# FrancisTheCat/raytracing_c

Measured on NVIDIA B200. Metric: Msamples/s (pixel*spp/s), helmet.glb 1920x1080, higher is better.
Workload: dtype f32

## Files before the change

### raytracing_c_b200/csrc/rt_stages.cuh

```cuda
#pragma once

#include <cuda_runtime.h>
#include <math_constants.h>

#include "rt_device.cuh"
#include "rt_fastdiv.h"
#include "rt_trace.cuh"
#include "rt_shade.cuh"

#if defined(RT_FAST) && RT_FAST
#define RT_KN(name) name##_fast
#else
#define RT_KN(name) name
#endif

#ifndef RT_TRACE_MIN_BLOCKS
#define RT_TRACE_MIN_BLOCKS 3
#endif
#ifndef RT_TRACE_MIN_BLOCKS_PRIMARY
#define RT_TRACE_MIN_BLOCKS_PRIMARY 4
#endif
#ifndef RT_TRACE_MIN_BLOCKS_WIDE
#define RT_TRACE_MIN_BLOCKS_WIDE 4
#endif
#ifndef RT_TRACE_WIDE_BOUNCES
#define RT_TRACE_WIDE_BOUNCES 2
#endif
#define RT_FULL 0xffffffffu
#ifndef RT_EMIT_ONE_ATOMIC
#define RT_EMIT_ONE_ATOMIC 1
#endif
#ifndef RT_BATCH_MAX
#define RT_BATCH_MAX 256u
#endif
#ifndef RT_ROOT_STEP_AT_REFILL
#define RT_ROOT_STEP_AT_REFILL 1
#endif

enum { Q_RAYS = 0, Q_FETCH = 1, Q_HITS = 2, Q_MISSES = 3, Q_STRIDE = 4 };

struct PathQueues {
  float4 *ray_a, *ray_b;
  float4 *hit_a, *hit_b, *hit_h;
  float4 *miss_a;
  float4 *tint, *emis;
  float4 *rad;
  unsigned *counts;
};

struct StageParams {
  SceneDev   scene;
  PathQueues q;
  int        width, height, tiles_x, tiles_y;
  int        split_rank, split_world, chunks_x;
  unsigned   n_tiles;
  int        sample0, n_samples;
  int        bounce, max_bounces;
  uint32_t   user_seed;
  unsigned   n_paths;
  RT_FastDiv div_samples, div_tiles_x, div_chunks_x;
  int        accumulate;
  float     *accum;
  float     *per_sample;
  int        per_sample_stride, per_sample_offset;
  int       *hit_ids;
  unsigned long long *counters;
  unsigned long long *counters_ex;
};

__device__ __forceinline__ float fract1(float v) { return v - floorf(v); }
__device__ __forceinline__ float hash12(float px, float py) {
  float a = fract1(px * 0.1031f);
  float b = fract1(py * 0.1031f);
  float c = fract1(px * 0.1031f);
  float k = 33.33f;
  float d = a * (b + k) + b * (c + k) + c * (a + k);
  return fract1((a + b + d * 2.0f) * (c + d));
}

__device__ __forceinline__ void tile_origin(const StageParams &P, unsigned tile, int &x0, int &y0) {
  if (P.split_world <= 1) {
    const unsigned row = rt_fastdiv(tile, P.div_tiles_x, (unsigned)P.tiles_x);
    x0 = (int)(tile - row * (unsigned)P.tiles_x) * 8;
    y0 = (int)row * 4;
  } else {
    const unsigned chunk = (tile >> 5) * (unsigned)P.split_world + (unsigned)P.split_rank, t = tile & 31u;
    const unsigned row = rt_fastdiv(chunk, P.div_chunks_x, (unsigned)P.chunks_x);
    x0 = (int)(chunk - row * (unsigned)P.chunks_x) * 32 + (int)(t & 3u) * 8;
    y0 = (int)row * 32 + (int)(t >> 2) * 4;
  }
}

#ifndef RT_PATH_LAYOUT
#define RT_PATH_LAYOUT 1
#endif
__device__ __forceinline__ void path_pixel(const StageParams &P, unsigned path, int &px, int &py, int &ls) {
#if RT_PATH_LAYOUT == 1
  const unsigned pix = rt_fastdiv(path, P.div_samples, (unsigned)P.n_samples);
  ls = (int)(path - pix * (unsigned)P.n_samples);
  const unsigned in_tile = pix & 31u, tile = pix >> 5;
#else
  unsigned in_tile = path & 31u, rest = path >> 5;
  unsigned tile = rest / (unsigned)P.n_samples;
  ls = (int)(rest - tile * (unsigned)P.n_samples);
#endif
  int x0, y0;
  tile_origin(P, tile, x0, y0);
  px = x0 + (int)(in_tile & 7u);
  py = y0 + (int)(in_tile >> 3);
}

__device__ __forceinline__ void add_counter(unsigned long long *counters, int k, unsigned v) {
  v += __shfl_xor_sync(RT_FULL, v, 16);
  v += __shfl_xor_sync(RT_FULL, v, 8);
  v += __shfl_xor_sync(RT_FULL, v, 4);
  v += __shfl_xor_sync(RT_FULL, v, 2);
  v += __shfl_xor_sync(RT_FULL, v, 1);
  if ((threadIdx.x & 31) == 0 && v) atomicAdd(&counters[k], (unsigned long long)v);
}

__device__ __forceinline__ unsigned warp_append(unsigned *count, bool want, unsigned lane) {
  const unsigned mask = __ballot_sync(RT_FULL, want);
  unsigned base = 0;
  if (lane == 0 && mask) base = atomicAdd(count, (unsigned)__popc(mask));
  base = __shfl_sync(RT_FULL, base, 0);
  return base + (unsigned)__popc(mask & ((1u << lane) - 1u));
}

#ifndef RT_MIN_BATCH
#define RT_MIN_BATCH 4u
#endif
#ifndef RT_REFILL_MIN_PRIMARY
#define RT_REFILL_MIN_PRIMARY 32
#endif
#ifndef RT_REFILL_MIN_BOUNCE
#define RT_REFILL_MIN_BOUNCE 20
#endif

template <bool PRIMARY, int MIN_BLOCKS = (PRIMARY ? RT_TRACE_MIN_BLOCKS_PRIMARY : RT_TRACE_MIN_BLOCKS)>
__global__ void __launch_bounds__(RT_BLOCK, MIN_BLOCKS)
RT_KN(rt_trace_kernel)(const __grid_constant__ StageParams P) {
  extern __shared__ float4 level_store[];
  const SceneDev &sc = P.scene;
  const unsigned lane = threadIdx.x & 31u;
  const unsigned lt_mask = (1u << lane) - 1u;
  float4 *levels = level_store + threadIdx.x;
  unsigned *counts = P.q.counts + P.bounce * Q_STRIDE;
  const unsigned n_in = PRIMARY ? P.n_paths : counts[Q_RAYS];
  unsigned c_rays = 0, c_nodes = 0, c_leaves = 0, c_accepts = 0, c_root_miss = 0;

  const float inv_w = 1.0f / (float)P.width, inv_h = 1.0f / (float)P.height;
  const float aspect = (float)P.width / (float)P.height;

  RayWalk w;
  w.flags = 0; w.leaf = -1; w.hit_slot = -1;
  bool     exhausted = false;
  unsigned q = 0, range_next = 0, range_end = 0;
  uint32_t seed0 = 0;
  const unsigned total_warps = gridDim.x * (RT_BLOCK / 32);
  unsigned batch = (n_in / (total_warps * 4u)) & ~31u;
  if (batch > RT_BATCH_MAX) batch = RT_BATCH_MAX;
  if (batch < 32u) {
    batch = (n_in + total_warps - 1u) / total_warps;
    if (batch < RT_MIN_BATCH) batch = RT_MIN_BATCH;
    if (batch > 32u) batch = 32u;
  }

  unsigned walking = 0;
  for (;;) {
    if (walking == 0 || (!exhausted && __popc(~walking) >= (PRIMARY ? RT_REFILL_MIN_PRIMARY : RT_REFILL_MIN_BOUNCE))) {
      const bool fin = (w.flags & (WALK_RAY | WALK_LIVE)) == WALK_RAY;
      const bool is_hit = fin && w.hit_slot >= 0;
      const bool is_miss = fin && w.hit_slot < 0;
      if (__any_sync(RT_FULL, fin)) {
        unsigned path = q;
        uint32_t rng = seed0;
        if (fin) {
          if (PRIMARY) {
            if (P.hit_ids) {
              int px, py, ls;
              path_pixel(P, q, px, py, ls);
              if (ls == 0) P.hit_ids[py * P.width + px] = w.hit_slot;
            }
          } else {
            const float4 b = P.q.ray_b[q];
            path = __float_as_uint(b.z);
            rng  = __float_as_uint(b.w);
          }
        }
#if RT_EMIT_ONE_ATOMIC
        const unsigned hmask = __ballot_sync(RT_FULL, is_hit), mmask = __ballot_sync(RT_FULL, is_miss);
        unsigned long long both = 0;
        if (lane == 0)
          both = atomicAdd(reinterpret_cast<unsigned long long *>(&counts[Q_HITS]),
                           (unsigned long long)__popc(hmask) | ((unsigned long long)__popc(mmask) << 32));
        both = __shfl_sync(RT_FULL, both, 0);
        const unsigned hpos = (unsigned)both + (unsigned)__popc(hmask & lt_mask);
        const unsigned mpos = (unsigned)(both >> 32) + (unsigned)__popc(mmask & lt_mask);
#else
        const unsigned hpos = warp_append(&counts[Q_HITS], is_hit, lane);
        const unsigned mpos = warp_append(&counts[Q_MISSES], is_miss, lane);
#endif
        if (is_hit) {
          P.q.hit_a[hpos] = make_float4(w.ox, w.oy, w.oz, w.dx);
          P.q.hit_b[hpos] = make_float4(w.dy, w.dz, __uint_as_float(path), __uint_as_float(rng));
          P.q.hit_h[hpos] = make_float4(w.hit_t, w.hit_u, w.hit_v, __int_as_float(w.hit_slot));
        }
        if (is_miss) {
          P.q.miss_a[mpos] = make_float4(w.dx, w.dy, w.dz, __uint_as_float(path));
        }
        if (fin) w.flags = 0;
      }
      if (!exhausted) {
        const unsigned idle = ~walking;
        if (range_next >= range_end) {
          unsigned base = 0;
          if (lane == 0) base = atomicAdd(&counts[Q_FETCH], batch);
          base = __shfl_sync(RT_FULL, base, 0);
          exhausted = base >= n_in;
          range_next = base;
          range_end = exhausted ? base : min(base + batch, n_in);
          if (batch > 32u) {
            const unsigned share = ((n_in - range_end) / (total_warps * 2u)) & ~31u;
            batch = share < 32u ? 32u : (share < batch ? share : batch);
          }
        }
        const unsigned take = min((unsigned)__popc(idle), range_end - range_next);
        const unsigned rank = (unsigned)__popc(idle & lt_mask);
        if ((idle >> lane & 1u) && rank < take) {
          q = range_next + rank;
          bool ok = true;
          float ox = 0, oy = 0, oz = 0, dx = 0, dy = 0, dz = -1;
          if (PRIMARY) {
            int px = 0, py = 0, ls = 0;
            path_pixel(P, q, px, py, ls);
            ok = px < P.width && py < P.height;
            if (ok) {
              const int s = P.sample0 + ls;
              float jit = hash12((float)px * 50.0f + (float)s, (float)py);
              float ux = ((float)px + jit - 0.5f) * 2.0f * inv_w - 1.0f;
              float uy = ((float)py + jit - 0.5f) * 2.0f * inv_h - 1.0f;
              float cx = ux * aspect, cy = -uy, cz = -sc.focal_length;
              float inv_len = 1.0f / __fsqrt_rn(cx * cx + cy * cy + cz * cz);
              dx = (sc.view[0][0] * cx + sc.view[0][1] * cy + sc.view[0][2] * cz) * inv_len;
              dy = (sc.view[1][0] * cx + sc.view[1][1] * cy + sc.view[1][2] * cz) * inv_len;
              dz = (sc.view[2][0] * cx + sc.view[2][1] * cy + sc.view[2][2] * cz) * inv_len;
              ox = sc.view[0][3]; oy = sc.view[1][3]; oz = sc.view[2][3];
              seed0 = rt_path_seed((uint32_t)(py * P.width + px), (uint32_t)s, P.user_seed);
            }
          } else {
            const float4 a = P.q.ray_a[q], b = P.q.ray_b[q];
            ox = a.x; oy = a.y; oz = a.z; dx = a.w; dy = b.x; dz = b.y;
          }
          if (ok) {
            walk_begin(w, sc, ox, oy, oz, dx, dy, dz);
            c_rays++;
            if (walk_misses_root<PRIMARY>(w, sc)) { w.flags = WALK_RAY; c_nodes++; c_root_miss++; }
#if RT_ROOT_STEP_AT_REFILL
            else walk_node_step<PRIMARY, true>(w, sc, levels, c_nodes);
#endif
          }
        }
        range_next += take;
      }
      walking = __ballot_sync(RT_FULL, w.flags & WALK_LIVE);
      if (walking == 0) {
        if (exhausted && __ballot_sync(RT_FULL, w.flags & WALK_RAY) == 0) break;
        continue;
      }
    }

    if (PRIMARY) {
      while ((w.flags & (WALK_LIVE | WALK_LEAF)) == WALK_LIVE) walk_node_step<PRIMARY>(w, sc, levels, c_nodes);
      __syncwarp();
      if (w.flags & WALK_LEAF) walk_leaf<PRIMARY>(w, sc, c_leaves, c_accepts);
    } else {
      const unsigned want_leaf = __ballot_sync(RT_FULL, w.flags & WALK_LEAF);
      if (2 * __popc(want_leaf) <= __popc(walking)) {
        if ((w.flags & (WALK_LIVE | WALK_LEAF)) == WALK_LIVE) walk_node_step<PRIMARY>(w, sc, levels, c_nodes);
      } else {
        if (w.flags & WALK_LEAF) walk_leaf<PRIMARY>(w, sc, c_leaves, c_accepts);
      }
    }
    walking = __ballot_sync(RT_FULL, w.flags & WALK_LIVE);
  }

  if (P.counters) {
    add_counter(P.counters, 0, c_rays);
    add_counter(P.counters, 1, c_nodes);
    add_counter(P.counters, 2, c_leaves);
    add_counter(P.counters, 3, c_accepts);
  }
  if (P.counters_ex) {
    add_counter(P.counters_ex, 0, c_root_miss);
    if (PRIMARY) add_counter(P.counters_ex, 1, c_rays);
  }
}

#ifndef RT_MISS_MIN_BLOCKS
#define RT_MISS_MIN_BLOCKS 8
#endif
__global__ void __launch_bounds__(256, RT_MISS_MIN_BLOCKS)
RT_KN(rt_miss_kernel)(const __grid_constant__ StageParams P) {
  const unsigned n = P.q.counts[P.bounce * Q_STRIDE + Q_MISSES];
  unsigned done = 0;
  for (unsigned i = blockIdx.x * blockDim.x + threadIdx.x; i < n; i += gridDim.x * blockDim.x) {
    const float4 a = P.q.miss_a[i];
    V3 env = environment(P.scene, mk3(a.x, a.y, a.z));
    V3 radiance;
    if (P.bounce == 0) {
      radiance = env;
    } else {
      const float4 t = P.q.tint[__float_as_uint(a.w)], e = P.q.emis[__float_as_uint(a.w)];
      radiance = add3(mul3(env, mk3(t.x, t.y, t.z)), mk3(e.x, e.y, e.z));
    }
    P.q.rad[__float_as_uint(a.w)] = make_float4(radiance.x, radiance.y, radiance.z, 0);
    done++;
  }
  if (P.counters) {
    add_counter(P.counters, 5, done);
    add_counter(P.counters, 7, done);
  }
}

__device__ __forceinline__ bool shade_hit(const SceneDev &sc, V3 &o, V3 &d, V3 &tint, V3 &emis,
                                          uint32_t &rng, float hit_t, float hit_u, float hit_v, int slot,
                                          unsigned &c_shades, unsigned &c_pass) {
  const float4 *rec = sc.tri_rec + (size_t)slot * 7;
  float4 r0 = __ldg(rec + 0), r1 = __ldg(rec + 1), r2 = __ldg(rec + 2);
  V3 ng = mk3(r0.x, r0.y, r0.z);
  V3 na = mk3(r0.w, r1.x, r1.y), nb = mk3(r1.z, r1.w, r2.x), nc = mk3(r2.y, r2.z, r2.w);
  float w1 = hit_u, w2 = hit_v, w0 = 1 - w1 - w2;
  V3 point  = add3(o, scale3(d, hit_t));
  V3 normal = mk3(na.x * w0 + nb.x * w1 + nc.x * w2,
                  na.y * w0 + nb.y * w1 + nc.y * w2,
                  na.z * w0 + nb.z * w1 + nc.z * w2);
  if (dot3(ng, d) > 0 || dot3(normal, d) > 0) {
    c_pass++;
    o = add3(point, scale3(d, RT_EPS));
    return true;
  }
  float4 r3 = __ldg(rec + 3), r4 = __ldg(rec + 4), r5 = __ldg(rec + 5), r6 = __ldg(rec + 6);
  ShadeIn in;
  in.dir = d;
  in.normal = normalize3(normal);
  in.normal_geo = ng;
  in.tangent   = mk3(r3.x, r3.y, r3.z);
  in.bitangent = mk3(r3.w, r4.x, r4.y);
  in.u = r4.z * w0 + r5.x * w1 + r5.z * w2;
  in.v = r4.w * w0 + r5.y * w1 + r5.w * w2;
  ShadeOut out;
  c_shades++;
  shade_pbr(sc, __float_as_int(r6.x), in, rng, out);
  emis = add3(emis, mul3(out.emission, tint));
  if (out.terminate) return false;
  d = out.dir;
  tint = mul3(tint, out.tint);
  float bias = (0.5f - (float)(dot3(ng, out.dir) < 0)) * 2.0f * RT_EPS;
  o = add3(point, scale3(ng, bias));
  return true;
}

#ifndef RT_SHADE_MIN_BLOCKS
#define RT_SHADE_MIN_BLOCKS 4
#endif
__global__ void __launch_bounds__(256, RT_SHADE_MIN_BLOCKS)
RT_KN(rt_shade_kernel)(const __grid_constant__ StageParams P) {
  const SceneDev &sc = P.scene;
  const unsigned lane = threadIdx.x & 31u;
  const unsigned n = P.q.counts[P.bounce * Q_STRIDE + Q_HITS];
  unsigned *next_rays = &P.q.counts[(P.bounce + 1) * Q_STRIDE + Q_RAYS];
  const unsigned n_round = (n + 31u) & ~31u;
  unsigned c_shades = 0, c_pass = 0, c_samples = 0;

  for (unsigned i = blockIdx.x * blockDim.x + threadIdx.x; i < n_round; i += gridDim.x * blockDim.x) {
    const bool active = i < n;
    bool  cont = false;
    V3    o = mk3(0, 0, 0), d = mk3(0, 0, 0), tint = mk3(0, 0, 0), emis = mk3(0, 0, 0);
    unsigned path = 0;
    uint32_t rng = 0;
    if (active) {
      const float4 a = P.q.hit_a[i], b = P.q.hit_b[i], h = P.q.hit_h[i];
      o = mk3(a.x, a.y, a.z); d = mk3(a.w, b.x, b.y);
      path = __float_as_uint(b.z); rng = __float_as_uint(b.w);
      tint = mk3(1, 1, 1); emis = mk3(0, 0, 0);
      if (P.bounce > 0) {
        const float4 c = P.q.tint[path], e = P.q.emis[path];
        tint = mk3(c.x, c.y, c.z); emis = mk3(e.x, e.y, e.z);
      }
      cont = shade_hit(sc, o, d, tint, emis, rng, h.x, h.y, h.z, __float_as_int(h.w), c_shades, c_pass);
      if (P.bounce + 1 >= P.max_bounces) cont = false;
      if (!cont) {
        P.q.rad[path] = make_float4(emis.x, emis.y, emis.z, 0);
        c_samples++;
      }
    }
    const unsigned pos = warp_append(next_rays, cont, lane);
    if (cont) {
      P.q.ray_a[pos] = make_float4(o.x, o.y, o.z, d.x);
      P.q.ray_b[pos] = make_float4(d.y, d.z, __uint_as_float(path), __uint_as_float(rng));
      P.q.tint[path] = make_float4(tint.x, tint.y, tint.z, 0);
      P.q.emis[path] = make_float4(emis.x, emis.y, emis.z, 0);
    }
  }
  if (P.counters) {
    add_counter(P.counters, 4, c_shades);
    add_counter(P.counters, 6, c_pass);
    add_counter(P.counters, 7, c_samples);
  }
}
```

### raytracing_c_b200/csrc/rt_trace.cuh

```cuda
#pragma once

#include <cuda_runtime.h>
#include <math_constants.h>

#include "rt_device.cuh"

#ifndef RT_BLOCK
#define RT_BLOCK 256
#endif


__device__ __forceinline__ float child_entry_any(float lox, float loy, float loz, float hix, float hiy, float hiz,
                                                 float ox, float oy, float oz, float ix, float iy, float iz, float t_max) {
  float ax = (lox - ox) * ix, ay = (loy - oy) * iy, az = (loz - oz) * iz;
  float bx = (hix - ox) * ix, by = (hiy - oy) * iy, bz = (hiz - oz) * iz;
  float nx = sel_min(ax, bx), ny = sel_min(ay, by), nz = sel_min(az, bz);
  float fx = sel_max(ax, bx), fy = sel_max(ay, by), fz = sel_max(az, bz);
  float enter = sel_max(RT_EPS, sel_max(nx, sel_max(ny, nz)));
  float leave = sel_min(t_max,  sel_min(fx, sel_min(fy, fz)));
  return (enter >= leave) ? CUDART_INF_F : enter;
}

template <bool REL>
__device__ __forceinline__ float child_entry_regular(float nx, float ny, float nz, float fx, float fy, float fz,
                                                     float ox, float oy, float oz, float ix, float iy, float iz, float t_max) {
#if defined(RT_FAST) && RT_FAST
  if (!REL) {
    float enter = fmaxf(fmaxf(fmaf(nx, ix, ox), fmaf(ny, iy, oy)), fmaxf(fmaf(nz, iz, oz), RT_EPS));
    float leave = fminf(fminf(fmaf(fx, ix, ox), fmaf(fy, iy, oy)), fminf(fmaf(fz, iz, oz), t_max));
    return (enter >= leave) ? CUDART_INF_F : enter;
  }
#endif
  if (!REL) { nx -= ox; ny -= oy; nz -= oz; fx -= ox; fy -= oy; fz -= oz; }
  float enter = fmaxf(fmaxf(nx * ix, ny * iy), fmaxf(nz * iz, RT_EPS));
  float leave = fminf(fminf(fx * ix, fy * iy), fminf(fz * iz, t_max));
  return (enter >= leave) ? CUDART_INF_F : enter;
}

#define RT_ROW_X_SUM  6u
#define RT_ROW_Y_SUM 10u
#define RT_ROW_Z_SUM 14u
template <bool REL>
__device__ __forceinline__ void node_entries_regular(const float4 *__restrict__ nb, unsigned onx, unsigned ony, unsigned onz,
                                                     float ox, float oy, float oz, float ix, float iy, float iz,
                                                     float t_max, float (&e)[8], bool upper = true) {
  const float4 *pnx = nb + onx, *pny = nb + ony, *pnz = nb + onz;
  const float4 *pfx = nb + (RT_ROW_X_SUM - onx), *pfy = nb + (RT_ROW_Y_SUM - ony), *pfz = nb + (RT_ROW_Z_SUM - onz);
  #pragma unroll
  for (int h = 0; h < 2; h++) {
    if (h == 1 && !upper) { e[4] = e[5] = e[6] = e[7] = CUDART_INF_F; break; }
    float4 nx = __ldg(pnx + h), ny = __ldg(pny + h), nz = __ldg(pnz + h);
    float4 fx = __ldg(pfx + h), fy = __ldg(pfy + h), fz = __ldg(pfz + h);
    e[4 * h + 0] = child_entry_regular<REL>(nx.x, ny.x, nz.x, fx.x, fy.x, fz.x, ox, oy, oz, ix, iy, iz, t_max);
    e[4 * h + 1] = child_entry_regular<REL>(nx.y, ny.y, nz.y, fx.y, fy.y, fz.y, ox, oy, oz, ix, iy, iz, t_max);
    e[4 * h + 2] = child_entry_regular<REL>(nx.z, ny.z, nz.z, fx.z, fy.z, fz.z, ox, oy, oz, ix, iy, iz, t_max);
    e[4 * h + 3] = child_entry_regular<REL>(nx.w, ny.w, nz.w, fx.w, fy.w, fz.w, ox, oy, oz, ix, iy, iz, t_max);
  }
}

struct Entries8 { float4 lo, hi; };
static __device__ __noinline__ Entries8 node_entries_any(const float4 *__restrict__ n4, float ox, float oy, float oz,
                                                  float ix, float iy, float iz, float t_max) {
  Entries8 r;
  {
    float4 lx = __ldg(n4 + 0), ly = __ldg(n4 + 2), lz = __ldg(n4 + 4), hx = __ldg(n4 + 6), hy = __ldg(n4 + 8), hz = __ldg(n4 + 10);
    r.lo.x = child_entry_any(lx.x, ly.x, lz.x, hx.x, hy.x, hz.x, ox, oy, oz, ix, iy, iz, t_max);
    r.lo.y = child_entry_any(lx.y, ly.y, lz.y, hx.y, hy.y, hz.y, ox, oy, oz, ix, iy, iz, t_max);
    r.lo.z = child_entry_any(lx.z, ly.z, lz.z, hx.z, hy.z, hz.z, ox, oy, oz, ix, iy, iz, t_max);
    r.lo.w = child_entry_any(lx.w, ly.w, lz.w, hx.w, hy.w, hz.w, ox, oy, oz, ix, iy, iz, t_max);
  }
  {
    float4 lx = __ldg(n4 + 1), ly = __ldg(n4 + 3), lz = __ldg(n4 + 5), hx = __ldg(n4 + 7), hy = __ldg(n4 + 9), hz = __ldg(n4 + 11);
    r.hi.x = child_entry_any(lx.x, ly.x, lz.x, hx.x, hy.x, hz.x, ox, oy, oz, ix, iy, iz, t_max);
    r.hi.y = child_entry_any(lx.y, ly.y, lz.y, hx.y, hy.y, hz.y, ox, oy, oz, ix, iy, iz, t_max);
    r.hi.z = child_entry_any(lx.z, ly.z, lz.z, hx.z, hy.z, hz.z, ox, oy, oz, ix, iy, iz, t_max);
    r.hi.w = child_entry_any(lx.w, ly.w, lz.w, hx.w, hy.w, hz.w, ox, oy, oz, ix, iy, iz, t_max);
  }
  return r;
}

__device__ __forceinline__ float min8(const float (&e)[8]) {
  return fminf(fminf(fminf(e[0], e[1]), fminf(e[2], e[3])), fminf(fminf(e[4], e[5]), fminf(e[6], e[7])));
}

#define RT_LEVELS(level, half) levels[(((level) - 2) * 2 + (half)) * RT_BLOCK]

#define WALK_RAY   1u
#define WALK_LIVE  2u
#define WALK_LEAF  4u
#define WALK_BOX   8u
#define WALK_REG  16u
struct RayWalk {
  float ox, oy, oz, dx, dy, dz, ix, iy, iz;
  float hit_t, hit_u, hit_v;
  int   hit_slot;
  int   node, level, leaf;
  unsigned pending, flags;
  unsigned onx, ony, onz;
  float e[8];
};

__device__ __forceinline__ void walk_begin(RayWalk &w, const SceneDev &sc, float ox, float oy, float oz,
                                           float dx, float dy, float dz) {
  w.ox = ox; w.oy = oy; w.oz = oz; w.dx = dx; w.dy = dy; w.dz = dz;
  w.ix = 1.0f / dx; w.iy = 1.0f / dy; w.iz = 1.0f / dz;
  const bool regular = (fabsf(w.ix) < CUDART_INF_F) & (fabsf(w.iy) < CUDART_INF_F) & (fabsf(w.iz) < CUDART_INF_F);
  w.onx = w.ix < 0.0f ? 6u : 0u; w.ony = w.iy < 0.0f ? 8u : 2u; w.onz = w.iz < 0.0f ? 10u : 4u;
  w.node = 0; w.level = sc.depth;
  w.pending = 0; w.leaf = -1;
  w.flags = WALK_RAY | WALK_LIVE | WALK_BOX | (regular ? WALK_REG : 0u);
  w.hit_t = CUDART_INF_F; w.hit_u = 0; w.hit_v = 0; w.hit_slot = -1;
}

template <bool REL>
__device__ __forceinline__ bool walk_misses_root(const RayWalk &w, const SceneDev &sc) {
  if (!(w.flags & WALK_REG)) return false;
  const bool negx = w.ix < 0.0f, negy = w.iy < 0.0f, negz = w.iz < 0.0f;
  const float nx = negx ? sc.root_hi[0] : sc.root_lo[0], fx = negx ? sc.root_lo[0] : sc.root_hi[0];
  const float ny = negy ? sc.root_hi[1] : sc.root_lo[1], fy = negy ? sc.root_lo[1] : sc.root_hi[1];
  const float nz = negz ? sc.root_hi[2] : sc.root_lo[2], fz = negz ? sc.root_lo[2] : sc.root_hi[2];
#if defined(RT_FAST) && RT_FAST
  return child_entry_regular<false>(nx, ny, nz, fx, fy, fz, -w.ox * w.ix, -w.oy * w.iy, -w.oz * w.iz, w.ix, w.iy, w.iz, CUDART_INF_F) == CUDART_INF_F;
#else
  return child_entry_regular<false>(nx, ny, nz, fx, fy, fz, w.ox, w.oy, w.oz, w.ix, w.iy, w.iz, CUDART_INF_F) == CUDART_INF_F;
#endif
}

template <bool REL, bool ROOT = false>
__device__ __forceinline__ void walk_node_step(RayWalk &w, const SceneDev &sc, float4 *levels, unsigned &c_nodes) {
  float (&e)[8] = w.e;
  for (;;) {
    if (w.flags & WALK_BOX) {
      if (w.flags & WALK_REG) {
        const bool upper = !ROOT || !sc.root_upper_empty;
        const size_t first = ROOT ? 0 : (size_t)w.node * 12;
        if (REL) node_entries_regular<true >((const float4 *)sc.nodes_rel + first, w.onx, w.ony, w.onz, 0, 0, 0, w.ix, w.iy, w.iz, w.hit_t, e, upper);
#if defined(RT_FAST) && RT_FAST
        else     node_entries_regular<false>((const float4 *)sc.nodes + first, w.onx, w.ony, w.onz, -w.ox * w.ix, -w.oy * w.iy, -w.oz * w.iz, w.ix, w.iy, w.iz, w.hit_t, e, upper);
#else
        else     node_entries_regular<false>((const float4 *)sc.nodes + first, w.onx, w.ony, w.onz, w.ox, w.oy, w.oz, w.ix, w.iy, w.iz, w.hit_t, e, upper);
#endif
      } else {
        const Entries8 r = node_entries_any((const float4 *)(sc.nodes + (size_t)w.node * 48), w.ox, w.oy, w.oz, w.ix, w.iy, w.iz, w.hit_t);
        e[0] = r.lo.x; e[1] = r.lo.y; e[2] = r.lo.z; e[3] = r.lo.w; e[4] = r.hi.x; e[5] = r.hi.y; e[6] = r.hi.z; e[7] = r.hi.w;
      }
      w.flags &= ~WALK_BOX;
      c_nodes++;
    }
    const float best = min8(e);
    if (!(best < w.hit_t)) {
      if (w.pending == 0) { w.flags &= ~WALK_LIVE; break; }
      const int up = __ffs(w.pending) - 1;
      w.pending &= w.pending - 1;
      #pragma unroll 1
      for (; w.level < up; w.level++) w.node = (w.node - 1) >> 3;
      float4 a = RT_LEVELS(w.level, 0), b = RT_LEVELS(w.level, 1);
      e[0] = a.x; e[1] = a.y; e[2] = a.z; e[3] = a.w; e[4] = b.x; e[5] = b.y; e[6] = b.z; e[7] = b.w;
      continue;
    }
    int pick = 7;
    #pragma unroll
    for (int j = 6; j >= 0; j--) pick = (e[j] == best) ? j : pick;
    #pragma unroll
    for (int j = 0; j < 8; j++) e[j] = (j == pick) ? CUDART_INF_F : e[j];
    const int child = 8 * w.node + 1 + pick;
    if (w.level == 1) { w.leaf = child - sc.n_internal; w.flags |= WALK_LEAF; break; }
    if (min8(e) < w.hit_t) {
      RT_LEVELS(w.level, 0) = make_float4(e[0], e[1], e[2], e[3]);
      RT_LEVELS(w.level, 1) = make_float4(e[4], e[5], e[6], e[7]);
      w.pending |= 1u << w.level;
    }
    w.node = child;
    w.level -= 1;
    w.flags |= WALK_BOX;
    break;
  }
}

template <bool REL>
__device__ __forceinline__ void leaf_triangle(RayWalk &w, const float4 A, const float4 B, const float4 C,
                                              const float4 *tq4, int slot) {
  const float e1x = A.w, e1y = B.x, e1z = B.y, e2x = B.z, e2y = B.w, e2z = C.x;
  float pvx = w.dy * e2z - w.dz * e2y, pvy = w.dz * e2x - w.dx * e2z, pvz = w.dx * e2y - w.dy * e2x;
  float det = e1x * pvx + e1y * pvy + e1z * pvz;
  float inv_det = 1.0f / det;
  float tvx = REL ? A.x : w.ox - A.x, tvy = REL ? A.y : w.oy - A.y, tvz = REL ? A.z : w.oz - A.z;
  float u = inv_det * (tvx * pvx + tvy * pvy + tvz * pvz);
  if (!((u < -RT_EPS) | (u > 1 + RT_EPS))) {
    float qvx, qvy, qvz, tq;
    if (REL) { qvx = C.y; qvy = C.z; qvz = C.w; tq = __ldg(&tq4->x); }
    else {
      qvx = tvy * e1z - tvz * e1y; qvy = tvz * e1x - tvx * e1z; qvz = tvx * e1y - tvy * e1x;
      tq = e2x * qvx + e2y * qvy + e2z * qvz;
    }
    float v = inv_det * (w.dx * qvx + w.dy * qvy + w.dz * qvz);
    float t = inv_det * tq;
    bool miss = (v < -RT_EPS) | (u + v > 1 + RT_EPS) | (t < RT_EPS);
    if (!miss && t > 0.0f && t < w.hit_t) { w.hit_t = t; w.hit_u = u; w.hit_v = v; w.hit_slot = slot; }
  }
}

template <bool REL>
__device__ __forceinline__ void walk_leaf(RayWalk &w, const SceneDev &sc, unsigned &c_leaves, unsigned &c_accepts) {
  const float t_before = w.hit_t;
  c_leaves++;
  if (!REL) {
    const float4 *tp = sc.tri_pos + (size_t)w.leaf * 24;
    float4 A0 = __ldg(tp), B0 = __ldg(tp + 1), C0 = __ldg(tp + 2);
    #pragma unroll 1
    for (int j = 0; j < 8; j += 2) {
      const float4 *odd = tp + 3 * (j + 1);
      const float4 A1 = __ldg(odd), B1 = __ldg(odd + 1), C1 = __ldg(odd + 2);
      leaf_triangle<false>(w, A0, B0, C0, nullptr, w.leaf * 8 + j);
      const float4 *even = tp + 3 * (j < 6 ? j + 2 : 7);
      A0 = __ldg(even); B0 = __ldg(even + 1); C0 = __ldg(even + 2);
      leaf_triangle<false>(w, A1, B1, C1, nullptr, w.leaf * 8 + j + 1);
    }
  } else {
    const float4 *tp = sc.tri_rel + (size_t)w.leaf * 32;
    #pragma unroll 1
    for (int j = 0; j < 8; j++) {
      const float4 A = __ldg(tp + 4 * j), B = __ldg(tp + 4 * j + 1), C = __ldg(tp + 4 * j + 2);
      leaf_triangle<true>(w, A, B, C, tp + 4 * j + 3, w.leaf * 8 + j);
    }
  }
  if (w.hit_t < t_before) c_accepts++;
  w.flags &= ~WALK_LEAF;
}
```

Before: 7235.

## Cull primary-ray leaf triangles with warp ray-bundle interval tests

For primary rays, each warp builds a bounding box of its live ray directions at refill time and stores it in shared memory. When lanes reach leaves, up to four distinct leaves per warp are tested cooperatively, one triangle per lane, using interval arithmetic over the direction box. This conservatively decides which triangles can be hit by any ray in the bundle, and lanes then intersect only the surviving candidates. It aims to skip triangle tests for coherent primary rays, at the cost of extra warp reductions, match/ballot operations and interval math on every leaf step. Leaves beyond the fourth distinct group still test all eight triangles.

New measurement: 7270 (median of 6 runs). Within noise of the previous version (+0.5%).

```diff
diff --git a/raytracing_c_b200/csrc/rt_stages.cuh b/raytracing_c_b200/csrc/rt_stages.cuh
--- a/raytracing_c_b200/csrc/rt_stages.cuh
+++ b/raytracing_c_b200/csrc/rt_stages.cuh
@@ -35,6 +35,14 @@
 #endif
 #ifndef RT_ROOT_STEP_AT_REFILL
 #define RT_ROOT_STEP_AT_REFILL 1
+#endif
+#ifndef RT_PRIMARY_BUNDLE
+#define RT_PRIMARY_BUNDLE 1
+#endif
+#if defined(RT_FAST) && RT_FAST
+#define RT_BUNDLE_ON 0
+#else
+#define RT_BUNDLE_ON RT_PRIMARY_BUNDLE
 #endif
 
 enum { Q_RAYS = 0, Q_FETCH = 1, Q_HITS = 2, Q_MISSES = 3, Q_STRIDE = 4 };
@@ -127,6 +135,47 @@
   return base + (unsigned)__popc(mask & ((1u << lane) - 1u));
 }
 
+__device__ __forceinline__ float4 *bundle_box_store() {
+  __shared__ float4 box[RT_BLOCK / 32][2];
+  return box[threadIdx.x >> 5];
+}
+
+__device__ __forceinline__ int float_key(float f) { const int k = __float_as_int(f); return k >= 0 ? k : k ^ 0x7fffffff; }
+__device__ __forceinline__ float key_float(int k) { return __int_as_float(k >= 0 ? k : k ^ 0x7fffffff); }
+
+__device__ __forceinline__ void bundle_refill(const RayWalk &w, float4 *box, unsigned lane) {
+  const bool live = w.flags & WALK_LIVE;
+  const int lx = __reduce_min_sync(RT_FULL, live ? float_key(w.dx) : INT_MAX), hx = __reduce_max_sync(RT_FULL, live ? float_key(w.dx) : INT_MIN);
+  const int ly = __reduce_min_sync(RT_FULL, live ? float_key(w.dy) : INT_MAX), hy = __reduce_max_sync(RT_FULL, live ? float_key(w.dy) : INT_MIN);
+  const int lz = __reduce_min_sync(RT_FULL, live ? float_key(w.dz) : INT_MAX), hz = __reduce_max_sync(RT_FULL, live ? float_key(w.dz) : INT_MIN);
+  if (lane == 0) {
+    box[0] = make_float4(key_float(lx), key_float(ly), key_float(lz), 0.0f);
+    box[1] = make_float4(key_float(hx), key_float(hy), key_float(hz), 0.0f);
+  }
+  __syncwarp();
+}
+
+__device__ __forceinline__ unsigned bundle_leaf_candidates(const RayWalk &w, const SceneDev &sc, const float4 *box,
+                                                           unsigned lane, unsigned &culled) {
+  const bool in_leaf = w.flags & WALK_LEAF;
+  const unsigned grp = __match_any_sync(RT_FULL, in_leaf ? w.leaf : -1);
+  const unsigned first = (unsigned)__ffs(grp) - 1u;
+  const unsigned leaders = __ballot_sync(RT_FULL, in_leaf && lane == first);
+  unsigned m = leaders;
+  #pragma unroll
+  for (unsigned k = 0; k < 3; k++) if (k < (lane >> 3)) m &= m - 1u;
+  const int leaf = __shfl_sync(RT_FULL, w.leaf, m ? __ffs(m) - 1 : 0);
+  const float T = __uint_as_float(__reduce_max_sync(RT_FULL, in_leaf ? __float_as_uint(w.hit_t) : 0u));
+  bool may = true;
+  if (m) may = bundle_triangle_may_hit(sc.tri_rel + (size_t)leaf * 32, (int)(lane & 7u), box, T);
+  const unsigned all = __ballot_sync(RT_FULL, may);
+  const unsigned g = (unsigned)__popc(leaders & ((1u << first) - 1u));
+  if (!in_leaf || g >= 4u) return 0xffu;
+  const unsigned cand = (all >> (8u * g)) & 0xffu;
+  culled += (unsigned)__popc(~cand & 0xffu);
+  return cand;
+}
+
 #ifndef RT_MIN_BATCH
 #define RT_MIN_BATCH 4u
 #endif
@@ -167,6 +216,9 @@
   }
 
   unsigned walking = 0;
+#if RT_BUNDLE_ON
+  unsigned c_culled = 0;
+#endif
   for (;;) {
     if (walking == 0 || (!exhausted && __popc(~walking) >= (PRIMARY ? RT_REFILL_MIN_PRIMARY : RT_REFILL_MIN_BOUNCE))) {
       const bool fin = (w.flags & (WALK_RAY | WALK_LIVE)) == WALK_RAY;
@@ -262,6 +314,9 @@
           }
         }
         range_next += take;
+#if RT_BUNDLE_ON
+        if (PRIMARY) bundle_refill(w, bundle_box_store(), lane);
+#endif
       }
       walking = __ballot_sync(RT_FULL, w.flags & WALK_LIVE);
       if (walking == 0) {
@@ -273,7 +328,14 @@
     if (PRIMARY) {
       while ((w.flags & (WALK_LIVE | WALK_LEAF)) == WALK_LIVE) walk_node_step<PRIMARY>(w, sc, levels, c_nodes);
       __syncwarp();
+#if RT_BUNDLE_ON
+      if (__any_sync(RT_FULL, w.flags & WALK_LEAF)) {
+        const unsigned cand = bundle_leaf_candidates(w, sc, bundle_box_store(), lane, c_culled);
+        if (w.flags & WALK_LEAF) walk_leaf_bundle(w, sc, c_leaves, c_accepts, cand);
+      }
+#else
       if (w.flags & WALK_LEAF) walk_leaf<PRIMARY>(w, sc, c_leaves, c_accepts);
+#endif
     } else {
       const unsigned want_leaf = __ballot_sync(RT_FULL, w.flags & WALK_LEAF);
       if (2 * __popc(want_leaf) <= __popc(walking)) {
@@ -294,6 +356,9 @@
   if (P.counters_ex) {
     add_counter(P.counters_ex, 0, c_root_miss);
     if (PRIMARY) add_counter(P.counters_ex, 1, c_rays);
+#if RT_BUNDLE_ON
+    if (PRIMARY) add_counter(P.counters_ex, 2, c_culled);
+#endif
   }
 }
 
diff --git a/raytracing_c_b200/csrc/rt_trace.cuh b/raytracing_c_b200/csrc/rt_trace.cuh
--- a/raytracing_c_b200/csrc/rt_trace.cuh
+++ b/raytracing_c_b200/csrc/rt_trace.cuh
@@ -200,6 +200,43 @@
   }
 }
 
+struct Ivl { float lo, hi; };
+__device__ __forceinline__ Ivl iv_mulc(Ivl a, float c) {
+  const float p = __fmul_rd(a.lo, c), q = __fmul_rd(a.hi, c), r = __fmul_ru(a.lo, c), s = __fmul_ru(a.hi, c);
+  return { fminf(p, q), fmaxf(r, s) };
+}
+__device__ __forceinline__ Ivl iv_mul(Ivl a, Ivl b) {
+  const float lo = fminf(fminf(__fmul_rd(a.lo, b.lo), __fmul_rd(a.lo, b.hi)), fminf(__fmul_rd(a.hi, b.lo), __fmul_rd(a.hi, b.hi)));
+  const float hi = fmaxf(fmaxf(__fmul_ru(a.lo, b.lo), __fmul_ru(a.lo, b.hi)), fmaxf(__fmul_ru(a.hi, b.lo), __fmul_ru(a.hi, b.hi)));
+  return { lo, hi };
+}
+__device__ __forceinline__ Ivl iv_add(Ivl a, Ivl b) { return { __fadd_rd(a.lo, b.lo), __fadd_ru(a.hi, b.hi) }; }
+__device__ __forceinline__ Ivl iv_sub(Ivl a, Ivl b) { return { __fsub_rd(a.lo, b.hi), __fsub_ru(a.hi, b.lo) }; }
+
+__device__ __forceinline__ bool bundle_triangle_may_hit(const float4 *__restrict__ tp, int j, const float4 *dbox, float T) {
+  const float4 A = __ldg(tp + 4 * j), B = __ldg(tp + 4 * j + 1), C = __ldg(tp + 4 * j + 2);
+  const float tq = __ldg(&tp[4 * j + 3].x);
+  const float4 lo = dbox[0], hi = dbox[1];
+  const float e1x = A.w, e1y = B.x, e1z = B.y, e2x = B.z, e2y = B.w, e2z = C.x;
+  const float big = fmaxf(fmaxf(fmaxf(fmaxf(fabsf(A.x), fabsf(A.y)), fmaxf(fabsf(A.z), fabsf(A.w))),
+                                fmaxf(fmaxf(fabsf(B.x), fabsf(B.y)), fmaxf(fabsf(B.z), fabsf(B.w)))),
+                          fmaxf(fmaxf(fmaxf(fabsf(C.x), fabsf(C.y)), fmaxf(fabsf(C.z), fabsf(C.w))), fabsf(tq)));
+  if (!(big < 0x1p60f)) return true;
+  const Ivl dx = { lo.x, hi.x }, dy = { lo.y, hi.y }, dz = { lo.z, hi.z };
+  const Ivl pvx = iv_sub(iv_mulc(dy, e2z), iv_mulc(dz, e2y));
+  const Ivl pvy = iv_sub(iv_mulc(dz, e2x), iv_mulc(dx, e2z));
+  const Ivl pvz = iv_sub(iv_mulc(dx, e2y), iv_mulc(dy, e2x));
+  const Ivl det = iv_add(iv_add(iv_mulc(pvx, e1x), iv_mulc(pvy, e1y)), iv_mulc(pvz, e1z));
+  if (!(det.lo > 0.0f || det.hi < 0.0f)) return true;
+  const Ivl inv = { __frcp_rd(det.hi), __frcp_ru(det.lo) };
+  if (!(fabsf(inv.lo) < CUDART_INF_F && fabsf(inv.hi) < CUDART_INF_F)) return true;
+  const Ivl u = iv_mul(inv, iv_add(iv_add(iv_mulc(pvx, A.x), iv_mulc(pvy, A.y)), iv_mulc(pvz, A.z)));
+  const Ivl v = iv_mul(inv, iv_add(iv_add(iv_mulc(dx, C.y), iv_mulc(dy, C.z)), iv_mulc(dz, C.w)));
+  const Ivl t = iv_mulc(inv, tq);
+  const Ivl uv = iv_add(u, v);
+  return !((u.hi < -RT_EPS) | (u.lo > 1 + RT_EPS) | (v.hi < -RT_EPS) | (uv.lo > 1 + RT_EPS) | (t.hi < RT_EPS) | (t.lo >= T));
+}
+
 template <bool REL>
 __device__ __forceinline__ void walk_leaf(RayWalk &w, const SceneDev &sc, unsigned &c_leaves, unsigned &c_accepts) {
   const float t_before = w.hit_t;
@@ -227,3 +264,18 @@
   if (w.hit_t < t_before) c_accepts++;
   w.flags &= ~WALK_LEAF;
 }
+
+__device__ __forceinline__ void walk_leaf_bundle(RayWalk &w, const SceneDev &sc, unsigned &c_leaves, unsigned &c_accepts,
+                                                 unsigned cand) {
+  const float t_before = w.hit_t;
+  c_leaves++;
+  const float4 *tp = sc.tri_rel + (size_t)w.leaf * 32;
+  #pragma unroll 1
+  for (unsigned m = cand; m; m &= m - 1u) {
+    const int j = __ffs(m) - 1;
+    const float4 A = __ldg(tp + 4 * j), B = __ldg(tp + 4 * j + 1), C = __ldg(tp + 4 * j + 2);
+    leaf_triangle<true>(w, A, B, C, tp + 4 * j + 3, w.leaf * 8 + j);
+  }
+  if (w.hit_t < t_before) c_accepts++;
+  w.flags &= ~WALK_LEAF;
+}
```
